# turtle-robotics/sea-current

Hardware: AMD Instinct MI355X
Metric: plans/sec (batched start-goal, 1024^2 grid) (higher is better)
Workload: dtype int32; 1 GPU; 1024x1024 random-obstacle grids (salt20, one grid and one query block per step), EDT + A*, 1024 batched queries per GPU and step, 10 steps = 10240 queries per library call; queries_per_launch=10240, map=salt20, queries_per_gpu=1024, queries_total=1024, lmax=4096, parallelism=query-sharded x1, contexts_in_flight=2, steps_per_call=10, hw_queues=4

## Files before the change

### sea-current_amd/csrc/astar.hip

```cpp
#include "sc_internal.h"
#include <stdlib.h>

#define NBUCKET 32
#ifndef ASTAR_CQ_THROUGHPUT
#define ASTAR_CQ_THROUGHPUT 1024
#define ASTAR_RU_THROUGHPUT 4
#endif
#ifndef ASTAR_CQ_LATENCY
#define ASTAR_CQ_LATENCY 2048
#define ASTAR_RU_LATENCY 8
#endif
#define E_RUN (1u << 18)
#define E_START (4u << 13 | 3u << 16)
#define RUNK 8
#ifndef WIDE_RUNS
#define WIDE_RUNS 0
#endif

struct astar_args {
    const uint8_t* moves;
    const int32_t* d2;
    int W, H;
    int32_t rmin;
    const int32_t* start;
    const int32_t* goal;
    const int32_t* qgrid;
    const int32_t* order;
    const int32_t* nq_dev;
    int nq;
    int Lmax;
    int32_t* path;
    int32_t* len;
    int32_t* cost;
    int32_t* status;
    void* g;
    uint32_t* closed;
    uint32_t* buckets;
    int cap;
    int32_t* expanded;
    int32_t* counter;
    int32_t* ovf_list;
    int32_t* ovf_count;
    int32_t* ovf_sticky;
    int nstat;
    int lazy;
    int tw, bw;
    size_t gcells, bwords;
};

__device__ __forceinline__ int octile(int x, int y, int gx, int gy) {
    int dx = abs(x - gx), dy = abs(y - gy);
    return 10 * max(dx, dy) + 4 * min(dx, dy);
}

__device__ __forceinline__ uint32_t gix(int x, int y, int tw) {
    return ((((uint32_t)(y >> 2) * (uint32_t)tw + (uint32_t)(x >> 2)) << 4) | ((uint32_t)(y & 3) << 2)) | (uint32_t)(x & 3);
}
__device__ __forceinline__ uint32_t gix8(int x, int y, int tw8) {
    return ((((uint32_t)(y >> 3) * (uint32_t)tw8 + (uint32_t)(x >> 3)) << 6) | ((uint32_t)(y & 7) << 3)) | (uint32_t)(x & 7);
}
template <typename GT> __device__ __forceinline__ uint32_t gidx(int x, int y, int tw);
template <> __device__ __forceinline__ uint32_t gidx<uint32_t>(int x, int y, int tw) { return gix(x, y, tw); }
template <> __device__ __forceinline__ uint32_t gidx<uint8_t>(int x, int y, int tw) { return gix8(x, y, tw); }
__device__ __forceinline__ uint32_t cix(int x, int y, int bw) {
    return (((uint32_t)(y >> 4) * (uint32_t)bw + (uint32_t)(x >> 5)) << 4) | (uint32_t)(y & 15);
}

template <typename T>
__device__ __forceinline__ T g_load(const T* p) {
    return __hip_atomic_load(p, __ATOMIC_RELAXED, __HIP_MEMORY_SCOPE_AGENT);
}

__device__ __forceinline__ uint32_t prune_always(int d) {
    const unsigned long long T = 0x75B6D9EA34C851A2ull;
    return (uint32_t)(T >> (8 * d)) & 0xFFu;
}

__device__ __forceinline__ uint32_t entry_pack(int x, int y, int d, uint32_t pmv) {
    const int e0 = (int)((0x6476u >> (4 * (d & 3))) & 7u), e1 = (int)((0x7554u >> (4 * (d & 3))) & 7u);
    const uint32_t side = d < 4 ? (((pmv >> e0) & 1u) | (((pmv >> e1) & 1u) << 1)) : 0u;
    return (uint32_t)y << 19 | side << 16 | (uint32_t)d << 13 | (uint32_t)x;
}
__device__ __forceinline__ uint32_t entry_prune(uint32_t e) {
    const int d = (int)((e >> 13) & 7u);
    uint32_t prune = prune_always(d);
    const int k0 = d < 2 ? 3 : 0, k1 = d < 2 ? 2 : 1;
    const int e0 = (int)((0x6476u >> (4 * (d & 3))) & 7u), e1 = (int)((0x7554u >> (4 * (d & 3))) & 7u);
    if ((e >> 16) & 1u) prune |= (1u << k0) | (1u << e0);
    if ((e >> 17) & 1u) prune |= (1u << k1) | (1u << e1);
    if (e & E_RUN) prune |= 1u << d;
    return (e & 0x3E000u) == E_START ? 0u : prune;
}

__device__ __forceinline__ void masked_atomic_or_issue(uint32_t* addr, uint32_t bits, uint32_t& old) {
    unsigned long long sv;
    asm volatile("s_mov_b64 %[sv], exec\n\t"
                 "v_cmp_ne_u32_e32 vcc, 0, %[b]\n\t"
                 "s_and_b64 exec, %[sv], vcc\n\t"
                 "global_atomic_or %[o], %[a], %[b], off sc0\n\t"
                 "s_mov_b64 exec, %[sv]"
                 : [sv] "=&s"(sv), [o] "+v"(old)
                 : [a] "v"(addr), [b] "v"(bits)
                 : "vcc", "scc", "memory");
}
__device__ __forceinline__ void atomic_wait(uint32_t& old) { asm volatile("s_waitcnt vmcnt(0)" : "+v"(old) : : "memory"); }
__device__ __forceinline__ void pop_pair_issue(const uint8_t* mv_addr, uint32_t* bit_addr, uint32_t bits, uint32_t& pmv, uint32_t& old) {
    unsigned long long sv;
    asm volatile("global_load_ubyte %[m], %[ma], off\n\t"
                 "s_mov_b64 %[sv], exec\n\t"
                 "v_cmp_ne_u32_e32 vcc, 0, %[b]\n\t"
                 "s_and_b64 exec, %[sv], vcc\n\t"
                 "global_atomic_or %[o], %[a], %[b], off sc0\n\t"
                 "s_mov_b64 exec, %[sv]"
                 : [sv] "=&s"(sv), [o] "+v"(old), [m] "=&v"(pmv)
                 : [a] "v"(bit_addr), [b] "v"(bits), [ma] "v"(mv_addr)
                 : "vcc", "scc", "memory");
}
__device__ __forceinline__ void pop_run_issue(const uint8_t* const (&ra)[RUNK - 1], const uint8_t* mv_addr, uint32_t* bit_addr, uint32_t bits,
                                              uint32_t (&rm)[RUNK - 1], uint32_t& pmv, uint32_t& old) {
    static_assert(RUNK == 8, "seven run loads are spelled out");
    unsigned long long sv;
    asm volatile("global_load_ubyte %[r0], %[p0], off\n\t"
                 "global_load_ubyte %[r1], %[p1], off\n\t"
                 "global_load_ubyte %[r2], %[p2], off\n\t"
                 "global_load_ubyte %[r3], %[p3], off\n\t"
                 "global_load_ubyte %[r4], %[p4], off\n\t"
                 "global_load_ubyte %[r5], %[p5], off\n\t"
                 "global_load_ubyte %[r6], %[p6], off\n\t"
                 "global_load_ubyte %[m], %[ma], off\n\t"
                 "s_mov_b64 %[sv], exec\n\t"
                 "v_cmp_ne_u32_e32 vcc, 0, %[b]\n\t"
                 "s_and_b64 exec, %[sv], vcc\n\t"
                 "global_atomic_or %[o], %[a], %[b], off sc0\n\t"
                 "s_mov_b64 exec, %[sv]"
                 : [sv] "=&s"(sv), [o] "+v"(old), [m] "=&v"(pmv), [r0] "=&v"(rm[0]), [r1] "=&v"(rm[1]), [r2] "=&v"(rm[2]), [r3] "=&v"(rm[3]),
                   [r4] "=&v"(rm[4]), [r5] "=&v"(rm[5]), [r6] "=&v"(rm[6])
                 : [a] "v"(bit_addr), [b] "v"(bits), [ma] "v"(mv_addr), [p0] "v"(ra[0]), [p1] "v"(ra[1]), [p2] "v"(ra[2]), [p3] "v"(ra[3]),
                   [p4] "v"(ra[4]), [p5] "v"(ra[5]), [p6] "v"(ra[6])
                 : "vcc", "scc", "memory");
}
__device__ __forceinline__ void pop_run_wait_loads(uint32_t (&rm)[RUNK - 1], uint32_t& pmv, uint32_t& old) {
    asm volatile("s_waitcnt vmcnt(1)" : "+v"(pmv), "+v"(old), "+v"(rm[0]), "+v"(rm[1]), "+v"(rm[2]), "+v"(rm[3]), "+v"(rm[4]), "+v"(rm[5]), "+v"(rm[6]) : : "memory");
}
__device__ __forceinline__ void run_loads_issue(const uint8_t* const (&ra)[RUNK - 1], uint32_t (&rm)[RUNK - 1]) {
    asm volatile("global_load_ubyte %[r0], %[p0], off\n\t"
                 "global_load_ubyte %[r1], %[p1], off\n\t"
                 "global_load_ubyte %[r2], %[p2], off\n\t"
                 "global_load_ubyte %[r3], %[p3], off\n\t"
                 "global_load_ubyte %[r4], %[p4], off\n\t"
                 "global_load_ubyte %[r5], %[p5], off\n\t"
                 "global_load_ubyte %[r6], %[p6], off"
                 : [r0] "=&v"(rm[0]), [r1] "=&v"(rm[1]), [r2] "=&v"(rm[2]), [r3] "=&v"(rm[3]), [r4] "=&v"(rm[4]), [r5] "=&v"(rm[5]), [r6] "=&v"(rm[6])
                 : [p0] "v"(ra[0]), [p1] "v"(ra[1]), [p2] "v"(ra[2]), [p3] "v"(ra[3]), [p4] "v"(ra[4]), [p5] "v"(ra[5]), [p6] "v"(ra[6])
                 : "memory");
}
__device__ __forceinline__ void run_loads_wait(uint32_t (&rm)[RUNK - 1]) {
    asm volatile("s_waitcnt vmcnt(0)" : "+v"(rm[0]), "+v"(rm[1]), "+v"(rm[2]), "+v"(rm[3]), "+v"(rm[4]), "+v"(rm[5]), "+v"(rm[6]) : : "memory");
}
__device__ __forceinline__ void atomic_wait_but(uint32_t& old, uint32_t (&rm)[RUNK - 1]) {
    asm volatile("s_waitcnt vmcnt(7)" : "+v"(old), "+v"(rm[0]), "+v"(rm[1]), "+v"(rm[2]), "+v"(rm[3]), "+v"(rm[4]), "+v"(rm[5]), "+v"(rm[6]) : : "memory");
}
__device__ __forceinline__ void pop_pair_wait_load(uint32_t& pmv, uint32_t& old) { asm volatile("s_waitcnt vmcnt(1)" : "+v"(pmv), "+v"(old) : : "memory"); }

__device__ __forceinline__ void pop_loads_issue(const uint8_t* mv_addr, const uint32_t* w_addr, uint32_t& byte, uint32_t& word) {
    asm volatile("global_load_ubyte %0, %2, off\n\t"
                 "global_load_dword %1, %3, off sc1"
                 : "=&v"(byte), "=&v"(word) : "v"(mv_addr), "v"(w_addr) : "memory");
}
__device__ __forceinline__ void pop_loads_wait(uint32_t& byte, uint32_t& word) { asm volatile("s_waitcnt vmcnt(0)" : "+v"(byte), "+v"(word) : : "memory"); }
__device__ __forceinline__ void masked_or_noret(uint32_t* addr, uint32_t bits) {
    unsigned long long sv;
    asm volatile("s_mov_b64 %[sv], exec\n\t"
                 "v_cmp_ne_u32_e32 vcc, 0, %[b]\n\t"
                 "s_and_b64 exec, %[sv], vcc\n\t"
                 "global_atomic_or %[a], %[b], off\n\t"
                 "s_mov_b64 exec, %[sv]"
                 : [sv] "=&s"(sv) : [a] "v"(addr), [b] "v"(bits) : "vcc", "scc", "memory");
}

__device__ __forceinline__ uint32_t bcast_group8(uint32_t v) {
    const uint32_t q = (uint32_t)__builtin_amdgcn_update_dpp(0, (int)v, 0x00 , 0xF, 0xF, false);
    const uint32_t r = (uint32_t)__builtin_amdgcn_update_dpp(0, (int)q, 0x114 , 0xF, 0xF, false);
    return q | r;
}

#ifdef ASTAR_MARKERS
#define MARK(i, v) do { if (threadIdx.x == 0 && blockIdx.x == 0) __hip_atomic_store(&a.counter[8 + (i)], (int)(v), __ATOMIC_RELAXED, __HIP_MEMORY_SCOPE_SYSTEM); } while (0)
#else
#define MARK(i, v) do { } while (0)
#endif
#ifdef ASTAR_STAMPS
#define STAMP(i) do { const unsigned long long t_ = __builtin_amdgcn_s_memtime(); stamp[i] += (long long)(t_ - t_last); t_last = t_; } while (0)
#else
#define STAMP(i) do { } while (0)
#endif

#ifndef HQ
#define HQ 256
#endif
#define ASTAR_SPIN_LIMIT (1 << 20)
template <typename GT, bool DUAL, int CQ, int REFILL_UNROLL>
__device__ __forceinline__ void astar_query(const astar_args& a, const int q, const int slot) {
    constexpr int REFILL = CQ / 2;
    __shared__ uint32_t qe[CQ + 64];
    __shared__ int s_head[NBUCKET];
    __shared__ int s_tail[NBUCKET];
    __shared__ uint32_t nd_xy[64];
    __shared__ uint32_t nd_mv[64];
    __shared__ uint16_t succ[512];
    __shared__ uint8_t prune_tbl[64];
    __shared__ uint32_t dup_tbl[DUAL ? 1024 + 64 : 1];
    __shared__ uint2 hq_rec[DUAL ? HQ + 64 : 1];
    __shared__ int hq_tail, hq_head, hq_clean, hq_stop, hq_ovf, hq_fcur, hq_found, hq_flush;
    constexpr int SCOPE = DUAL ? __HIP_MEMORY_SCOPE_WORKGROUP : __HIP_MEMORY_SCOPE_WAVEFRONT;
    const int lane = threadIdx.x & 63;
    const int wv = DUAL ? __builtin_amdgcn_readfirstlane((int)(threadIdx.x >> 6)) : 0;
    const int W = a.W, H = a.H;
    const size_t cells = (size_t)W * H;
    const int s = a.start[q], t = a.goal[q];
    int32_t* path = a.path + (size_t)q * a.Lmax;

    int out_st = SC_Q_OK, out_len = 0, out_cost = -1, nexp = 0, npop = 0, kcyc = 0, nstep = 0;
    const size_t grid_off = a.qgrid ? (size_t)a.qgrid[q] * cells : 0;
    const uint8_t* const mvs = a.moves + grid_off;
    const bool bad = s < 0 || t < 0 || (size_t)s >= cells || (size_t)t >= cells || a.d2[grid_off + s] < a.rmin || a.d2[grid_off + t] < a.rmin;
    if (bad) out_st = SC_Q_BAD_ENDPOINT;
    else if (s == t) {
        if (lane == 0 && wv == 0) path[0] = s;
        out_len = 1; out_cost = 0; nexp = 1;
    } else {
    MARK(0, 1);
    const int tw = a.tw, bw = a.bw;
    GT* g = static_cast<GT*>(a.g) + (size_t)slot * a.gcells;
    uint32_t* cl = a.closed + (size_t)slot * a.bwords;
    uint32_t* bk = a.buckets + (size_t)slot * NBUCKET * a.cap;
    const int cap = a.cap, capm = a.cap - 1;
    const int sx = s % W, sy = s / W, gx = t % W, gy = t / W;
    const int ddx[8] = {1, -1, 0, 0, 1, -1, 1, -1};
    const int ddy[8] = {0, 0, 1, -1, 1, 1, -1, -1};

    {
        uint4* p = reinterpret_cast<uint4*>(cl);
        const size_t n4 = a.bwords >> 2;
        for (size_t i = DUAL ? threadIdx.x : lane; i < n4; i += DUAL ? 128 : 64) p[i] = make_uint4(0, 0, 0, 0);
    }
    __builtin_amdgcn_wave_barrier();
    if (wv == 0 && lane < NBUCKET) { s_head[lane] = 0; s_tail[lane] = 0; }
    if (wv == 0) prune_tbl[lane] = (uint8_t)entry_prune((uint32_t)lane << 13);
    if (DUAL)
        for (int i = threadIdx.x; i < 1024 + 64; i += 128) dup_tbl[i] = 0xFFFFFFFFu;
    int fcur = octile(sx, sy, gx, gy);
    if (wv == 0 && lane == 0) {
        qe[0] = (uint32_t)sy << 19 | E_START | (uint32_t)sx;
        hq_tail = 0; hq_head = 0; hq_clean = 0; hq_stop = 0; hq_ovf = 0; hq_fcur = fcur; hq_found = 0; hq_flush = 0;
    }
    asm volatile("s_waitcnt vmcnt(0)" ::: "memory");
    wave_lds_sync();
    if (DUAL) __syncthreads();
    int lh = 0, lt = 1;
    MARK(0, 2);

    bool found = false, ovf = false;
    const unsigned long long t_begin = __builtin_amdgcn_s_memtime();
#ifdef ASTAR_STAMPS
    long long stamp[12] = {0, 0, 0, 0, 0, 0, 0, 0, 0, 0, 0, 0};
    unsigned long long t_last = t_begin;
    int nwide = 0, nrounds = 0, n_qfull = 0, n_lvl = 0, b_batches = 0, b_records = 0, b_idle = 0, n_refill = 0;
#endif
    int steps_left = (int)(8 * cells + 1024 < 0x7FFFFFFF ? 8 * cells + 1024 : 0x7FFFFFFF);

    const int mdx = (int)((0x2252u >> (2 * (lane & 7))) & 3u) - 1;
    const int mdy = (int)((0x0A25u >> (2 * (lane & 7))) & 3u) - 1;
    const uint32_t mw = (lane & 7) < 4 ? 10u : 14u;
    const int moff = mdy * W + mdx;

    auto push_entry = [&](const bool act, const uint32_t ne, const int df) {
        const bool same = act && df == 0;
        const unsigned long long m0 = __ballot(same);
        bool spill = false;
        if (m0) {
            const int cnt = __popcll(m0);
            if (__builtin_expect(lt - lh + cnt <= CQ, 1)) {
                if (same) {
                    const int rank = __builtin_amdgcn_mbcnt_hi((uint32_t)(m0 >> 32), __builtin_amdgcn_mbcnt_lo((uint32_t)m0, 0u));
                    qe[(lt + rank) & (CQ - 1)] = ne;
                }
                lt += cnt;
            } else spill = true;
        }
        if (act && (df != 0 || spill)) {
            const int bb = (fcur + df) & 31;
            const int pos = __hip_atomic_fetch_add(&s_tail[bb], 1, __ATOMIC_RELAXED, SCOPE);
            if (__builtin_expect(pos - __hip_atomic_load(&s_head[bb], __ATOMIC_RELAXED, SCOPE) >= cap, 0)) ovf = true;
            else bk[(size_t)bb * cap + (pos & capm)] = ne;
        }
        lt = __builtin_amdgcn_readfirstlane(lt);
    };
    int hq_tl = 0, hq_hd = 0;
    auto hand_over = [&](const bool rec, const int hx, const int hy, const uint32_t hm, const uint32_t hp) {
        const unsigned long long wm = __ballot(rec);
        if (wm) {
            const int cnt = __popcll(wm);
            int waited = 0;
            while (__builtin_expect(hq_tl + cnt - hq_hd > HQ, 0)) {
                hq_hd = __builtin_amdgcn_readfirstlane(__hip_atomic_load(&hq_head, __ATOMIC_RELAXED, SCOPE));
                if (hq_tl + cnt - hq_hd > HQ) {
                    __builtin_amdgcn_s_sleep(1);
#ifdef ASTAR_STAMPS
                    ++n_qfull;
#endif
                    if (++waited > ASTAR_SPIN_LIMIT) {
                        ovf = true; steps_left = -1;
                        return wm;
                    }
                }
            }
            {
                const int r = (hq_tl + (int)__builtin_amdgcn_mbcnt_hi((uint32_t)(wm >> 32), __builtin_amdgcn_mbcnt_lo((uint32_t)wm, 0u))) & (HQ - 1);
                hq_rec[rec ? r : HQ + lane] = make_uint2((uint32_t)hy << 16 | (uint32_t)hx, hm | hp << 8);
            }
            hq_tl += cnt;
            wave_lds_sync();
            __hip_atomic_store(&hq_tail, hq_tl, __ATOMIC_RELAXED, SCOPE);
        }
        return wm;
    };
    constexpr uint32_t DUP_KEY = 0x1FFF1FFFu, DUP_EMPTY = 0xFFFFFFFFu;
    auto dup_settle = [&](const bool is, const int hx, const int hy, const uint32_t he) {
        const int h = is ? ((hx + 32 * hy) & 1023) : 1024 + lane;
        const uint32_t key = (uint32_t)hy << 16 | (uint32_t)hx;
        const uint32_t mine = key | ((uint32_t)(lane & 7) << 13) | ((uint32_t)(lane >> 3) << 29);
        const uint32_t before = dup_tbl[h];
        __builtin_amdgcn_fence(__ATOMIC_ACQ_REL, "wavefront");
        dup_tbl[h] = mine;
        wave_lds_sync();
        const uint32_t now = dup_tbl[h];
        const bool closed_before = is && before != DUP_EMPTY && ((before ^ key) & DUP_KEY) == 0u;
        int res = closed_before ? 1 : 0;
        if (__ballot(is && now != mine)) {
            if (is && !closed_before && now != mine) res = ((now ^ key) & DUP_KEY) == 0u ? 1 : 2;
            const bool back = res == 2;
            const unsigned long long mb = __ballot(back);
            if (mb) {
                const int c = __popcll(mb);
                if (__builtin_expect(lt - lh + c <= CQ, 1)) {
                    qe[back ? ((lt + (int)__builtin_amdgcn_mbcnt_hi((uint32_t)(mb >> 32), __builtin_amdgcn_mbcnt_lo((uint32_t)mb, 0u))) & (CQ - 1)) : CQ + lane] = he;
                    lt += c;
                } else push_entry(back, he, 0);
                npop -= c;
            }
        }
        wave_lds_sync();
        return res;
    };
    if (DUAL && wv == 1) {
        int hd = 0;
        bool dirty = false;
        for (;;) {
            const int tl = __builtin_amdgcn_readfirstlane(__hip_atomic_load(&hq_tail, __ATOMIC_RELAXED, SCOPE));
            const int stop = __builtin_amdgcn_readfirstlane(__hip_atomic_load(&hq_stop, __ATOMIC_RELAXED, SCOPE));
            wave_lds_sync();
            if (tl == hd) {
                if (dirty) {
                    asm volatile("s_waitcnt vmcnt(0)" ::: "memory");
                    if (lane == 0) __hip_atomic_store(&hq_clean, hd, __ATOMIC_RELAXED, SCOPE);
                    dirty = false;
                }
                if (stop) break;
                __builtin_amdgcn_s_sleep(4);
#ifdef ASTAR_STAMPS
                ++b_idle;
#endif
                continue;
            }
            if (a.lazy && tl - hd < 48 && !stop &&
                __builtin_amdgcn_readfirstlane(__hip_atomic_load(&hq_flush, __ATOMIC_RELAXED, SCOPE)) != tl) {
                __builtin_amdgcn_s_sleep(4);
                continue;
            }
#ifdef ASTAR_STAMPS
            ++b_batches; b_records += min(tl - hd, 64);
#endif
            const int n = min(tl - hd, 64);
            const bool valid = lane < n;
            const int r = (hd + lane) & (HQ - 1);
            const uint2 rec = valid ? hq_rec[r] : make_uint2(0u, 0u);
            const uint32_t xy = rec.x, m = rec.y;
            const uint32_t f = (uint32_t)__builtin_amdgcn_readfirstlane(__hip_atomic_load(&hq_fcur, __ATOMIC_RELAXED, SCOPE));
            hd += n;
            wave_lds_sync();
            if (lane == 0) __hip_atomic_store(&hq_head, hd, __ATOMIC_RELAXED, SCOPE);
            dirty = true;
            const int x = xy & 0xFFFF, y = xy >> 16;
            const int hc = octile(x, y, gx, gy);
            if (valid) g[gidx<GT>(x, y, tw)] = (GT)(f - (uint32_t)hc);
            if (__ballot(valid && x == gx && y == gy) && lane == 0) __hip_atomic_store(&hq_found, 1, __ATOMIC_RELAXED, SCOPE);
            uint32_t mv = m & 0xFFu;
            nd_xy[lane] = xy;
            nd_mv[lane] = ((m >> 8) & 0xFFu) | ((f - (uint32_t)hc) << 8);
            const uint32_t cnt = (uint32_t)__popc(mv);
            int base = 0, total = 0;
#pragma unroll
            for (int bb = 0; bb < 4; ++bb) {
                const unsigned long long mm = __ballot((cnt >> bb) & 1u);
                base += (int)__builtin_amdgcn_mbcnt_hi((uint32_t)(mm >> 32), __builtin_amdgcn_mbcnt_lo((uint32_t)mm, 0u)) << bb;
                total += __popcll(mm) << bb;
            }
            while (mv) {
                const int dd = __ffs((int)mv) - 1;
                mv &= mv - 1;
                succ[base++] = (uint16_t)(lane << 3 | dd);
            }
            wave_lds_sync();
            for (int j0 = 0; j0 < total; j0 += 64) {
                const bool act = j0 + lane < total;
                const uint32_t sd = act ? succ[j0 + lane] : 0u;
                const int par = (int)(sd >> 3), d = (int)(sd & 7u);
                const uint32_t pxy = nd_xy[par], pm = nd_mv[par];
                const int px = pxy & 0xFFFF, py = pxy >> 16;
                const int nx = px + (int)((0x2252u >> (2 * d)) & 3u) - 1, ny = py + (int)((0x0A25u >> (2 * d)) & 3u) - 1;
                const uint32_t fs = (pm >> 8) + (d < 4 ? 10u : 14u) + (uint32_t)octile(nx, ny, gx, gy);
                if (act) {
                    const int bb = (int)(fs & 31u);
                    const int pos = __hip_atomic_fetch_add(&s_tail[bb], 1, __ATOMIC_RELAXED, SCOPE);
                    if (pos - __hip_atomic_load(&s_head[bb], __ATOMIC_RELAXED, SCOPE) >= cap) __hip_atomic_store(&hq_ovf, 1, __ATOMIC_RELAXED, SCOPE);
                    else bk[(size_t)bb * cap + (pos & capm)] = entry_pack(nx, ny, d, pm & 0xFFu);
                }
            }
            wave_lds_sync();
        }
#ifdef ASTAR_STAMPS
        if (lane == 0 && a.Lmax >= 32) { path[16] = b_batches; path[17] = b_records; path[18] = b_idle; }
#endif
    } else {
    for (;;) {
        const int b = fcur & 31;
        const uint32_t* bq = bk + (size_t)b * cap;
        for (;;) {
            if (__builtin_expect(lt == lh, 0)) {
                STAMP(0);
                wave_lds_sync();
                const int hd = __builtin_amdgcn_readfirstlane(__hip_atomic_load(&s_head[b], __ATOMIC_RELAXED, SCOPE));
                const int tl = __builtin_amdgcn_readfirstlane(__hip_atomic_load(&s_tail[b], __ATOMIC_RELAXED, SCOPE));
                if (hd == tl) break;
                const int n = min(tl - hd, REFILL);
                for (int base = lane; base < n; base += 64 * REFILL_UNROLL) {
                    uint32_t chunk[REFILL_UNROLL];
#pragma unroll
                    for (int k = 0; k < REFILL_UNROLL; ++k)
                        if (base + 64 * k < n) chunk[k] = bq[(hd + base + 64 * k) & capm];
#pragma unroll
                    for (int k = 0; k < REFILL_UNROLL; ++k)
                        if (base + 64 * k < n) qe[(lt + base + 64 * k) & (CQ - 1)] = chunk[k];
                }
                lt += n;
                if (lane == 0) __hip_atomic_store(&s_head[b], hd + n, __ATOMIC_RELAXED, SCOPE);
                wave_lds_sync();
                STAMP(10);
#ifdef ASTAR_STAMPS
                ++n_refill;
#endif
            }
            const int n = min(64, lt - lh);
            npop += n; ++nstep;
            STAMP(0);
            if (DUAL && n <= 16) {
                const int kl = n <= 4 ? 3 : n <= 8 ? 2 : n <= 16 ? 1 : 0, KL = 1 << kl, GL = 2 * KL;
                const int sub = lane >> (kl + 1), j = (lane >> kl) & 1, k = lane & (KL - 1);
                const bool valid = sub < n;
                const uint32_t e_raw = qe[(lh + sub) & (CQ - 1)];
                const uint32_t e = valid ? e_raw : 0u;
                lh += n;
                const int x = e & 0x1FFF, y = e >> 19;
                const uint32_t bit = 1u << (x & 31);
                const int dxg = gx - x, dyg = gy - y, adx = abs(dxg), ady = abs(dyg);
                const int dD = 4 + ((dxg < 0 ? 1 : 0) | (dyg < 0 ? 2 : 0));
                const int dS = adx > ady ? (dxg < 0 ? 1 : 0) : (dyg < 0 ? 3 : 2);
                const uint32_t bD = adx >= 1 && ady >= 1 ? 1u << dD : 0u, bS = adx != ady ? 1u << dS : 0u;
                const int d = j ? dS : dD;
                const bool has = valid && (j ? bS : bD) != 0u;
                const int lgeom = j ? abs(adx - ady) : min(adx, ady);
                const int ddx_ = (int)((0x2252u >> (2 * d)) & 3u) - 1, ddy_ = (int)((0x0A25u >> (2 * d)) & 3u) - 1;
                const uint8_t* const addr = mvs + (y * W + x) + (has ? min(k, lgeom - 1) : 0) * (ddy_ * W + ddx_);
                const bool head = valid && j == 0 && k == 0;
                uint32_t old, byte;
                uint32_t* const wa = &cl[cix(x, y, bw)];
                pop_loads_issue(addr, wa, byte, old);
                const uint32_t prune = prune_tbl[(e >> 13) & 63u];
                const int dup = dup_settle(head, x, y, e);
                pop_loads_wait(byte, old);
                const bool link = has && k < lgeom && ((byte >> d) & 1u) && (k > 0 || !((prune >> d) & 1u));
                const unsigned long long lm = __ballot(link);
                const uint32_t grp = (uint32_t)(lm >> (lane & ~(KL - 1))) & ((1u << KL) - 1u);
                const int run = __ffs((int)~grp) - 1;
                const uint32_t ne = entry_pack(x + (k + 1) * ddx_, y + (k + 1) * ddy_, d, byte) | (k + 1 < run ? E_RUN : 0u);
                const bool won1 = head && dup == 0 && !(old & bit);
                masked_or_noret(wa, won1 ? bit : 0u);
                const unsigned long long wm1 = __ballot(won1);
                const bool act = ((wm1 >> (lane & ~(GL - 1))) & 1ull) && k < run;
                {
                    const unsigned long long ma = __ballot(act);
                    if (ma) {
                        const int c = __popcll(ma);
                        if (__builtin_expect(lt - lh + c <= CQ, 1)) {
                            qe[act ? ((lt + (int)__builtin_amdgcn_mbcnt_hi((uint32_t)(ma >> 32), __builtin_amdgcn_mbcnt_lo((uint32_t)ma, 0u))) & (CQ - 1)) : CQ + lane] = ne;
                            lt += c;
                        } else push_entry(act, ne, 0);
                    }
                }
                hand_over(won1, x, y, (byte & ~prune) & ~(bD | bS), byte);
                nexp += __popcll(wm1);
                STAMP(8);
            } else if (!DUAL && n <= 8) {
                const int sub = lane >> 3, d = lane & 7;
                const bool valid = sub < n;
                const uint32_t e = valid ? qe[(lh + sub) & (CQ - 1)] : 0u;
                lh += n;
                const int x = e & 0x1FFF, y = e >> 19;
                const uint32_t bit = 1u << (x & 31);
                uint32_t old = 0, pmv;
                const int hc = octile(x, y, gx, gy);
                const int nx = x + mdx, ny = y + mdy;
                const int df = (int)mw + octile(nx, ny, gx, gy) - hc;
                const int adx = abs(gx - x), ady = abs(gy - y);
                const int lgeom = d >= 4 ? min(adx, ady) : abs(adx - ady);
                const int lmax = valid && df == 0 ? min(RUNK, lgeom) : 1;
                const uint8_t* const cell = mvs + (y * W + x);
                const uint8_t* ra[RUNK - 1];
                uint32_t rm[RUNK - 1];
#pragma unroll
                for (int k = 1; k < RUNK; ++k) ra[k - 1] = cell + min(k, lmax - 1) * moff;
                pop_run_issue(ra, cell, &cl[cix(x, y, bw)], valid && d == 0 ? bit : 0u, rm, pmv, old);
                const uint32_t prune = prune_tbl[(e >> 13) & 63u];
                pop_run_wait_loads(rm, pmv, old);
                const bool cand = valid && (((pmv & ~prune) >> d) & 1u);
                int run = cand ? 1 : 0;
#pragma unroll
                for (int k = 1; k < RUNK; ++k)
                    if (run == k && k < lmax && ((rm[k - 1] >> d) & 1u)) run = k + 1;
                const uint32_t ne = entry_pack(nx, ny, d, pmv) | (run > 1 ? E_RUN : 0u);
                atomic_wait(old);
                old = bcast_group8(old);
                const bool won = valid && !(old & bit);
                push_entry(won && cand, ne, df);
#pragma unroll
                for (int k = 2; k <= RUNK; ++k) {
                    if (__ballot(won && run >= k) == 0) break;
                    push_entry(won && run >= k, entry_pack(x + k * mdx, y + k * mdy, d, rm[k - 2]) | (run > k ? E_RUN : 0u), 0);
                }
                nexp += __popcll(__ballot(won && d == 0));
                if (__ballot(won && x == gx && y == gy)) found = true;
                if (won && d == 0) g[gidx<GT>(x, y, tw)] = (GT)(fcur - hc);
                STAMP(8);
            } else if (DUAL) {
#ifdef ASTAR_STAMPS
                ++nwide;
#endif
                const bool valid = lane < n;
                const uint32_t e_raw = qe[(lh + lane) & (CQ - 1)];
                const uint32_t e = valid ? e_raw : 0u;
                lh += n;
                const int x = e & 0x1FFF, y = e >> 19;
                const uint32_t bit = 1u << (x & 31);
                uint32_t old, pmv;
                uint32_t* const wa = &cl[cix(x, y, bw)];
                pop_loads_issue(mvs + (y * W + x), wa, pmv, old);
                const int dup = dup_settle(valid, x, y, e);
                const uint32_t prune = prune_tbl[(e >> 13) & 63u];
                const int dxg = gx - x, dyg = gy - y, adx = abs(dxg), ady = abs(dyg);
                const int dD = 4 + ((dxg < 0 ? 1 : 0) | (dyg < 0 ? 2 : 0));
                const int dS = adx > ady ? (dxg < 0 ? 1 : 0) : (dyg < 0 ? 3 : 2);
                const uint32_t bD = adx >= 1 && ady >= 1 ? 1u << dD : 0u, bS = adx != ady ? 1u << dS : 0u;
                const int nxD = x + (dxg < 0 ? -1 : 1), nyD = y + (dyg < 0 ? -1 : 1);
                const int nxS = x + (adx > ady ? (dxg < 0 ? -1 : 1) : 0), nyS = y + (adx > ady ? 0 : (dyg < 0 ? -1 : 1));
                pop_loads_wait(pmv, old);
                const uint32_t cand = valid ? (pmv & ~prune) : 0u;
                const uint32_t neD = (uint32_t)nyD << 19 | (uint32_t)dD << 13 | (uint32_t)nxD;
                const uint32_t neS = entry_pack(nxS, nyS, dS, pmv);
                const bool won = valid && dup == 0 && !(old & bit);
                masked_or_noret(wa, won ? bit : 0u);
                {
                    const bool pD = won && (cand & bD), pS = won && (cand & bS);
                    const unsigned long long mD = __ballot(pD), mS = __ballot(pS);
                    const int cD = __popcll(mD), c2 = cD + __popcll(mS);
                    if (c2) {
                        if (__builtin_expect(lt - lh + c2 <= CQ, 1)) {
                            qe[pD ? ((lt + (int)__builtin_amdgcn_mbcnt_hi((uint32_t)(mD >> 32), __builtin_amdgcn_mbcnt_lo((uint32_t)mD, 0u))) & (CQ - 1)) : CQ + lane] = neD;
                            qe[pS ? ((lt + cD + (int)__builtin_amdgcn_mbcnt_hi((uint32_t)(mS >> 32), __builtin_amdgcn_mbcnt_lo((uint32_t)mS, 0u))) & (CQ - 1)) : CQ + lane] = neS;
                            lt += c2;
                        } else {
                            push_entry(pD, neD, 0);
                            push_entry(pS, neS, 0);
                        }
                    }
                }
                nexp += __popcll(hand_over(won, x, y, cand & ~(bD | bS), pmv));
                STAMP(6);
            } else {
                STAMP(0);
                const bool valid = lane < n;
                const uint32_t e = valid ? qe[(lh + lane) & (CQ - 1)] : 0u;
                lh += n;
                const int x = e & 0x1FFF, y = e >> 19;
                const uint32_t bit = 1u << (x & 31);
                uint32_t old = 0, pmv;
                pop_pair_issue(mvs + (y * W + x), &cl[cix(x, y, bw)], valid ? bit : 0u, pmv, old);
                const uint32_t prune = prune_tbl[(e >> 13) & 63u];
                const int hc = octile(x, y, gx, gy);
                STAMP(1);
                pop_pair_wait_load(pmv, old);
                STAMP(2);
                uint32_t mv = valid ? (pmv & ~prune) : 0u;
                nd_xy[lane] = (uint32_t)y << 16 | (uint32_t)x;
                nd_mv[lane] = pmv;
                const uint32_t cnt = (uint32_t)__popc(mv);
                int base = 0, total = 0;
#pragma unroll
                for (int bb = 0; bb < 4; ++bb) {
                    const unsigned long long m = __ballot((cnt >> bb) & 1u);
                    base += (int)__builtin_amdgcn_mbcnt_hi((uint32_t)(m >> 32), __builtin_amdgcn_mbcnt_lo((uint32_t)m, 0u)) << bb;
                    total += __popcll(m) << bb;
                }
                while (mv) {
                    const int dd = __ffs((int)mv) - 1;
                    mv &= mv - 1;
                    succ[base++] = (uint16_t)(lane << 3 | dd);
                }
                wave_lds_sync();
                STAMP(3);
                bool won = false;
#ifdef ASTAR_STAMPS
                ++nwide;
#endif
                for (int j0 = 0; j0 < total; j0 += 64) {
#ifdef ASTAR_STAMPS
                    ++nrounds;
#endif
                    const bool act = j0 + lane < total;
                    const uint32_t sd = act ? succ[j0 + lane] : 0u;
                    const int par = (int)(sd >> 3), d = (int)(sd & 7u);
                    const uint32_t xy = nd_xy[par], pmvp = nd_mv[par];
                    const int px = xy & 0xFFFF, py = xy >> 16;
                    const int ddx_ = (int)((0x2252u >> (2 * d)) & 3u) - 1, ddy_ = (int)((0x0A25u >> (2 * d)) & 3u) - 1;
                    const int nx = px + ddx_, ny = py + ddy_;
                    const int df = (d < 4 ? 10 : 14) + octile(nx, ny, gx, gy) - octile(px, py, gx, gy);
                    const int adx = abs(gx - px), ady = abs(gy - py);
                    const int lgeom = d >= 4 ? min(adx, ady) : abs(adx - ady);
                    const int lmax = WIDE_RUNS && act && df == 0 ? min(RUNK, lgeom) : 1;
                    const int so = ddy_ * W + ddx_;
                    const uint8_t* const cell = mvs + (py * W + px);
                    const uint8_t* ra[RUNK - 1];
                    uint32_t rm[RUNK - 1];
#pragma unroll
                    for (int k = 1; k < RUNK; ++k) ra[k - 1] = cell + min(k, lmax - 1) * so;
                    if (WIDE_RUNS) run_loads_issue(ra, rm);
                    if (j0 == 0) {
                        STAMP(4);
                        if (WIDE_RUNS) atomic_wait_but(old, rm); else atomic_wait(old);
                        STAMP(5);
                        won = valid && !(old & bit);
                        nexp += __popcll(__ballot(won));
                        if (__ballot(won && x == gx && y == gy)) found = true;
                        nd_mv[lane] = pmv | (won ? 0x100u : 0u);
                        wave_lds_sync();
                    }
                    const bool go = act && ((nd_mv[par] >> 8) & 1u);
                    int run = 1;
                    if (WIDE_RUNS) {
                        run_loads_wait(rm);
#pragma unroll
                        for (int k = 1; k < RUNK; ++k)
                            if (run == k && k < lmax && ((rm[k - 1] >> d) & 1u)) run = k + 1;
                    }
                    push_entry(go, entry_pack(nx, ny, d, pmvp) | (run > 1 ? E_RUN : 0u), df);
                    if (WIDE_RUNS) {
#pragma unroll
                        for (int k = 2; k <= RUNK; ++k) {
                            if (__ballot(go && run >= k) == 0) break;
                            push_entry(go && run >= k, entry_pack(px + k * ddx_, py + k * ddy_, d, rm[k - 2]) | (run > k ? E_RUN : 0u), 0);
                        }
                    }
                }
                if (total == 0) {
                    atomic_wait(old);
                    won = valid && !(old & bit);
                    nexp += __popcll(__ballot(won));
                    if (__ballot(won && x == gx && y == gy)) found = true;
                }
                if (won) g[gidx<GT>(x, y, tw)] = (GT)(fcur - hc);
                STAMP(6);
            }
            lt = __builtin_amdgcn_readfirstlane(lt);
            lh = __builtin_amdgcn_readfirstlane(lh);
            nexp = __builtin_amdgcn_readfirstlane(nexp);
            found = __builtin_amdgcn_readfirstlane((int)found) != 0;
            wave_lds_sync();
            MARK(1, steps_left); MARK(2, fcur); MARK(3, nexp); MARK(4, lt - lh);
            if (--steps_left < 0) ovf = true;
            if (__builtin_expect(DUAL ? steps_left < 0 : __ballot(ovf) != 0, 0)) break;
        }
        if (DUAL) {
            STAMP(0);
            if (a.lazy && lane == 0) __hip_atomic_store(&hq_flush, hq_tl, __ATOMIC_RELAXED, SCOPE);
            for (int waited = 0; __builtin_amdgcn_readfirstlane(__hip_atomic_load(&hq_clean, __ATOMIC_RELAXED, SCOPE)) != hq_tl;) {
                __builtin_amdgcn_s_sleep(1);
#ifdef ASTAR_STAMPS
                ++n_lvl;
#endif
                if (++waited > ASTAR_SPIN_LIMIT) { ovf = true; break; }
            }
            wave_lds_sync();
            if (__hip_atomic_load(&hq_ovf, __ATOMIC_RELAXED, SCOPE)) ovf = true;
            if (__builtin_amdgcn_readfirstlane(__hip_atomic_load(&hq_found, __ATOMIC_RELAXED, SCOPE))) found = true;
            STAMP(7);
        }
        if (__ballot(ovf) || found) break;
        const int rh = __hip_atomic_load(&s_head[lane & 31], __ATOMIC_RELAXED, __HIP_MEMORY_SCOPE_WAVEFRONT);
        const int rt = __hip_atomic_load(&s_tail[lane & 31], __ATOMIC_RELAXED, __HIP_MEMORY_SCOPE_WAVEFRONT);
        const uint32_t nonempty = (uint32_t)__ballot(lane < NBUCKET && rh != rt);
        if (nonempty == 0) break;
        const int r0 = (fcur + 1) & 31;
        const uint32_t rot = r0 ? (nonempty >> r0) | (nonempty << (32 - r0)) : nonempty;
        fcur += 1 + (__ffs((int)rot) - 1);
        if (DUAL && lane == 0) __hip_atomic_store(&hq_fcur, fcur, __ATOMIC_RELAXED, SCOPE);
        STAMP(9);
    }
    if (DUAL && lane == 0) __hip_atomic_store(&hq_stop, 1, __ATOMIC_RELAXED, SCOPE);
    }
    if (DUAL) __syncthreads();

    const bool overflow = __ballot(ovf) != 0;
    if (overflow) {
        if (lane == 0 && wv == 0) {
            const int i = atomicAdd(a.ovf_count, 1);
            a.ovf_list[i] = q;
            *a.ovf_sticky = 1;
        }
        out_st = SC_Q_RING_OVERFLOW;
    } else if (!found) {
        out_st = SC_Q_NO_PATH;
    } else {
        STAMP(9);
        asm volatile("s_waitcnt vmcnt(0)" ::: "memory");
        const int Lmax = a.Lmax;
        int cx = gx, cy = gy, L = 1;
        uint32_t gc = (uint32_t)fcur;
        if (lane == 0) path[Lmax - 1] = t;
        bool broken = false;
        const int wox = lane % 7 - 3, woy = lane / 7 - 3;
        const int md = lane & 7;
        const int mdx_ = (int)((0x2252u >> (2 * md)) & 3u) - 1, mdy_ = (int)((0x0A25u >> (2 * md)) & 3u) - 1;
        const uint32_t mw_ = md < 4 ? 10u : 14u;
        while (!broken && (cx != sx || cy != sy)) {
            uint32_t info = 0u, gw = 0u;
            {
                const int nx = cx + wox, ny = cy + woy;
                if (lane < 49 && nx >= 0 && ny >= 0 && nx < W && ny < H) {
                    const uint32_t mvb = mvs[ny * W + nx];
                    const uint32_t cw = g_load(&cl[cix(nx, ny, bw)]);
                    gw = (uint32_t)g_load(&g[gidx<GT>(nx, ny, tw)]);
                    info = mvb | ((cw >> (nx & 31)) & 1u) << 8;
                }
            }
            int ox = 0, oy = 0;
            for (int k = 0; k < 3 && !broken && (cx != sx || cy != sy); ++k) {
                const int src = (oy - mdy_ + 3) * 7 + (ox - mdx_ + 3);
                const uint32_t ni = (uint32_t)__shfl((int)info, src, 64), ng = (uint32_t)__shfl((int)gw, src, 64);
                const bool ok = lane < 8 && ((ni >> md) & 1u) && ((ni >> 8) & 1u) && (GT)ng == (GT)(gc - mw_);
                const unsigned long long m = __ballot(ok);
                if (!m) broken = true;
                else {
                    const int d = __ffsll((long long)m) - 1;
                    cx -= ddx[d]; cy -= ddy[d];
                    ox -= ddx[d]; oy -= ddy[d];
                    gc -= (d < 4 ? 10u : 14u);
                    ++L;
                    if (lane == 0 && L <= Lmax) path[Lmax - L] = cy * W + cx;
                }
            }
        }
        if (broken) out_st = SC_Q_NO_PATH;
        else if (L > Lmax) { out_st = SC_Q_TRUNCATED; out_len = L; out_cost = fcur; }
        else {
            const int shift = Lmax - L;
            if (shift > 0) {
                __builtin_amdgcn_fence(__ATOMIC_RELEASE, "workgroup");
                for (int i = 0; i < L; i += 64) {
                    int v = 0;
                    if (i + lane < L) v = __hip_atomic_load(&path[shift + i + lane], __ATOMIC_RELAXED, __HIP_MEMORY_SCOPE_AGENT);
                    if (i + lane < L) path[i + lane] = v;
                    __builtin_amdgcn_fence(__ATOMIC_RELEASE, "workgroup");
                }
            }
            out_len = L; out_cost = fcur;
        }
        STAMP(11);
    }
    kcyc = (int)((__builtin_amdgcn_s_memtime() - t_begin) >> 10);
#ifdef ASTAR_STAMPS
    if (lane == 0 && wv == 0 && a.Lmax >= 16) {
        for (int i = 0; i < 12; ++i) path[i] = (int)(stamp[i] >> 10);
        path[12] = nwide; path[13] = nrounds; path[14] = n_qfull; path[15] = n_lvl; path[19] = n_refill;
    }
#endif
    }
    if (lane == 0 && wv == 0) {
        a.status[q] = out_st; a.len[q] = out_len; a.cost[q] = out_cost;
        a.expanded[q] = nexp; a.expanded[a.nstat + q] = npop; a.expanded[2 * a.nstat + q] = kcyc; a.expanded[3 * a.nstat + q] = nstep;
    }
}

template <typename GT>
__global__ void __launch_bounds__(64) astar_kernel(astar_args a) {
    const int nq = a.nq_dev ? *a.nq_dev : a.nq;
    for (;;) {
        const int qi = __builtin_amdgcn_readfirstlane(atomicAdd(a.counter, 1)) >> 6;
        if (qi >= nq) break;
        astar_query<GT, false, ASTAR_CQ_THROUGHPUT, ASTAR_RU_THROUGHPUT>(a, a.order ? a.order[qi] : qi, (int)blockIdx.x);
    }
}

template <typename GT, int CQ, int RU>
__global__ void __launch_bounds__(128) astar_kernel_dual(astar_args a) {
    __shared__ int s_qi;
    const int nq = a.nq_dev ? *a.nq_dev : a.nq;
    for (;;) {
        if (threadIdx.x == 0) s_qi = atomicAdd(a.counter, 64) >> 6;
        __syncthreads();
        const int qi = __builtin_amdgcn_readfirstlane(s_qi);
        __syncthreads();
        if (qi >= nq) break;
        astar_query<GT, true, CQ, RU>(a, a.order ? a.order[qi] : qi, (int)blockIdx.x);
        __syncthreads();
    }
}

__global__ void __launch_bounds__(1024) astar_prep_kernel(const int32_t* __restrict__ start, const int32_t* __restrict__ goal, int Q, int W,
                                                          int H, int32_t* __restrict__ order, int32_t* __restrict__ ctr) {
    __shared__ int hist[1024];
    __shared__ int scan[1024];
    const int tid = threadIdx.x;
    if (tid < 4) ctr[tid] = 0;
    if (!order) return;
    hist[tid] = 0;
    __syncthreads();
    const int hmax = 14 * max(W, H) + 1;
    auto key = [&](int q) {
        const int s = start[q], t = goal[q];
        if (s < 0 || t < 0 || s >= W * H || t >= W * H) return 1023;
        const int h = octile(s % W, s / W, t % W, t / W);
        return 1023 - min(1023, (int)(((long long)h * 1024) / hmax));
    };
    for (int q = tid; q < Q; q += 1024) atomicAdd(&hist[key(q)], 1);
    __syncthreads();
    scan[tid] = hist[tid];
    __syncthreads();
    for (int o = 1; o < 1024; o <<= 1) {
        const int v = tid >= o ? scan[tid - o] : 0;
        __syncthreads();
        scan[tid] += v;
        __syncthreads();
    }
    hist[tid] = scan[tid] - hist[tid];
    __syncthreads();
    for (int q = tid; q < Q; q += 1024) order[atomicAdd(&hist[key(q)], 1)] = q;
}

__global__ void __launch_bounds__(256) gfield_kernel(const uint32_t* g, const uint32_t* cl, int W, int H, int tw, int bw, uint32_t* out) {
    size_t i = (size_t)blockIdx.x * 256 + threadIdx.x;
    if (i < (size_t)W * H) {
        const int x = (int)(i % W), y = (int)(i / W);
        out[i] = (cl[cix(x, y, bw)] >> (x & 31)) & 1u ? g[gix(x, y, tw)] : 0xFFFFFFFFu;
    }
}

static int astar_resident_waves(sc_ctx* ctx) {
    if (ctx->astar_waves > 0) return ctx->astar_waves;
    int per_cu = 0, dev = ctx->device;
    hipDeviceProp_t prop;
    if (hipOccupancyMaxActiveBlocksPerMultiprocessor(&per_cu, astar_kernel<uint8_t>, 64, 0) != hipSuccess || per_cu <= 0) per_cu = 8;
    if (hipGetDeviceProperties(&prop, dev) != hipSuccess || prop.multiProcessorCount <= 0) prop.multiProcessorCount = 256;
    int w = per_cu * prop.multiProcessorCount;
    if (const char* e = getenv("SC_ASTAR_WAVES")) { const int v = atoi(e); if (v > 0) w = v; }
    ctx->astar_waves = w;
    return w;
}
static int astar_resident_dual(sc_ctx* ctx, bool latency) {
    int& cached = latency ? ctx->astar_dual_lat : ctx->astar_dual;
    if (cached >= 0) return cached;
    int per_cu = 0, n = 0;
    hipDeviceProp_t prop;
    const hipError_t e_ = latency ? hipOccupancyMaxActiveBlocksPerMultiprocessor(&per_cu, astar_kernel_dual<uint8_t, ASTAR_CQ_LATENCY, ASTAR_RU_LATENCY>, 128, 0)
                                  : hipOccupancyMaxActiveBlocksPerMultiprocessor(&per_cu, astar_kernel_dual<uint8_t, ASTAR_CQ_THROUGHPUT, ASTAR_RU_THROUGHPUT>, 128, 0);
    if (e_ == hipSuccess && per_cu > 0 && hipGetDeviceProperties(&prop, ctx->device) == hipSuccess && prop.multiProcessorCount > 0)
        n = per_cu * prop.multiProcessorCount;
    if (const char* e = getenv("SC_ASTAR_DUAL")) { const int v = atoi(e); if (v == 0) n = 0; else if (v > 1 && v < n) n = v; }
    if (latency) { if (const char* e = getenv("SC_ASTAR_LATENCY")) { if (atoi(e) == 0) n = 0; } }
    cached = n;
    return n;
}

static int astar_run(sc_ctx* ctx, const int32_t* d2, int G, const int32_t* qgrid, int W, int H, int32_t r2, const int32_t* start,
                     const int32_t* goal, int Q, int Lmax, int32_t* path, int32_t* len, int32_t* cost,
                     int32_t* status, bool full_g = false) {
    const size_t cells = (size_t)W * H;
    const int tw = full_g ? (W + 3) >> 2 : (W + 7) >> 3, bw = (W + 31) >> 5;
    const size_t gcells = full_g ? (size_t)tw * ((H + 3) >> 2) * 16 : (size_t)tw * ((H + 7) >> 3) * 64;
    const size_t gsz = full_g ? 4 : 1;
    const size_t bwords = (size_t)bw * ((H + 15) >> 4) * 16;
    const int32_t rmin = r2 > 1 ? r2 : 1;
    int r = sc_scratch_reserve(ctx, &ctx->moves, cells * (size_t)G);
    if (r != SC_OK) return r;
    r = sc_launch_moves(ctx, d2, W, H * G, H, r2, (uint8_t*)ctx->moves.p);
    if (r != SC_OK) return r;
    r = sc_scratch_reserve(ctx, &ctx->qstats, (size_t)Q * 6 * sizeof(int32_t));
    if (r != SC_OK) return r;
    int32_t* expanded = (int32_t*)ctx->qstats.p;
    int32_t* order = expanded + 4 * (size_t)Q;
    int32_t* ovf_list = order + Q;
    ctx->last_Q = Q;
    int cap = ctx->astar_cap;
    if (const char* e = getenv("SC_ASTAR_CAP")) { const int v = atoi(e); if (v >= 1024 && (v & (v - 1)) == 0) cap = v; }
    if (cells > ((size_t)1 << 21)) {
        int want = 1 << 15;
        while (want < 64 * (W > H ? W : H)) want <<= 1;
        if (cap < want) cap = want;
    }
    const size_t per_slot = gcells * gsz + bwords * 4 + (size_t)NBUCKET * cap * 4;
    size_t slots = ctx->astar_slot_budget / per_slot;
    const size_t rlat = (size_t)astar_resident_dual(ctx, true);
    const bool latency = !full_g && rlat > 0 && (size_t)Q <= rlat && (size_t)Q <= slots;
    const size_t rdual = latency ? rlat : (size_t)astar_resident_dual(ctx, false);
    const bool dual = !full_g && rdual > 0;
    const size_t resident = dual ? rdual : (size_t)astar_resident_waves(ctx);
    if (slots > resident) slots = resident;
    if (slots > (size_t)Q) slots = Q;
    if (slots < 1) slots = 1;
    auto ring_slots = [](size_t n) { return n > 16 ? n : (size_t)16; };
    if (slots * gcells * gsz > ctx->gslots.bytes || slots * bwords * 4 > ctx->closed.bytes || ring_slots(slots) * NBUCKET * (size_t)cap * 4 > ctx->buckets.bytes) {
        size_t free_b = 0, total_b = 0;
        if (hipMemGetInfo(&free_b, &total_b) == hipSuccess) {
            const size_t avail = (size_t)(0.9 * (double)(free_b + ctx->gslots.bytes + ctx->closed.bytes + ctx->buckets.bytes));
            while (slots > 1 && slots * (gcells * gsz + bwords * 4) + ring_slots(slots) * NBUCKET * (size_t)cap * 4 > avail) slots = (slots + 1) / 2;
        }
    }
    for (;;) {
        r = sc_scratch_reserve(ctx, &ctx->gslots, slots * gcells * gsz);
        if (r == SC_OK) r = sc_scratch_reserve(ctx, &ctx->closed, slots * bwords * 4);
        if (r == SC_OK) r = sc_scratch_reserve(ctx, &ctx->buckets, ring_slots(slots) * NBUCKET * (size_t)cap * 4);
        if (r == SC_OK) break;
        if (r != SC_ERR_NOMEM || slots <= 1) return r;
        (void)hipGetLastError();
        slots = (slots + 1) / 2;
    }
    if (!ctx->actr.p) {
        r = sc_scratch_reserve(ctx, &ctx->actr, 16 * sizeof(int32_t));
        if (r != SC_OK) return r;
        SC_HIP(ctx, hipMemsetAsync(ctx->actr.p, 0, 16 * sizeof(int32_t), ctx->stream));
    }
    int32_t* ctr = (int32_t*)ctx->actr.p;

    const bool sorted = (size_t)Q > slots;
    int tk = sc_time_begin(ctx, SC_K_ASTAR);
    hipLaunchKernelGGL(astar_prep_kernel, dim3(1), dim3(1024), 0, ctx->stream, start, goal, Q, W, H, sorted ? order : (int32_t*)nullptr, ctr);
    astar_args a{(const uint8_t*)ctx->moves.p, d2, W, H, rmin, start, goal, qgrid, sorted ? order : nullptr, nullptr, Q, Lmax, path, len,
                 cost, status, ctx->gslots.p, (uint32_t*)ctx->closed.p, (uint32_t*)ctx->buckets.p, cap, expanded, ctr,
                 ovf_list, ctr + 1, ctr + 4, Q, (dual && (size_t)Q > slots) ? 1 : 0, tw, bw, gcells, bwords};
    if (full_g) hipLaunchKernelGGL(astar_kernel<uint32_t>, dim3((unsigned)slots), dim3(64), 0, ctx->stream, a);
    else if (dual && latency && (size_t)Q <= slots)
        hipLaunchKernelGGL((astar_kernel_dual<uint8_t, ASTAR_CQ_LATENCY, ASTAR_RU_LATENCY>), dim3((unsigned)slots), dim3(128), 0, ctx->stream, a);
    else if (dual)
        hipLaunchKernelGGL((astar_kernel_dual<uint8_t, ASTAR_CQ_THROUGHPUT, ASTAR_RU_THROUGHPUT>), dim3((unsigned)slots), dim3(128), 0, ctx->stream, a);
    else hipLaunchKernelGGL(astar_kernel<uint8_t>, dim3((unsigned)slots), dim3(64), 0, ctx->stream, a);
    {
        const size_t rslots = slots >= 16 ? slots / 16 : 1;
        const int rcap = cap * 16;
        astar_args b = a;
        b.order = ovf_list; b.nq_dev = ctr + 1; b.nq = 0; b.cap = rcap; b.counter = ctr + 2;
        b.ovf_list = order; b.ovf_count = ctr + 3;
        if (full_g) hipLaunchKernelGGL(astar_kernel<uint32_t>, dim3((unsigned)rslots), dim3(64), 0, ctx->stream, b);
        else hipLaunchKernelGGL(astar_kernel<uint8_t>, dim3((unsigned)rslots), dim3(64), 0, ctx->stream, b);
    }
    sc_time_end(ctx, tk);
    SC_HIP(ctx, hipGetLastError());
    return SC_OK;
}

extern "C" int sc_astar_batch(sc_ctx* ctx, const int32_t* d2, int W, int H, int32_t r2_clear,
                              const int32_t* start, const int32_t* goal, int Q, int Lmax,
                              int32_t* path, int32_t* len, int32_t* cost, int32_t* status) {
    if (!ctx || !d2 || !start || !goal || !path || !len || !cost || !status || W <= 0 || H <= 0 || Q < 0 ||
        Lmax <= 0 || W > SC_MAX_DIM || H > SC_MAX_DIM)
        return SC_ERR_INVALID;
    if (Q == 0) return SC_OK;
    SC_HIP(ctx, hipSetDevice(ctx->device));
    return astar_run(ctx, d2, 1, nullptr, W, H, r2_clear, start, goal, Q, Lmax, path, len, cost, status);
}

extern "C" int sc_astar_batch_multi(sc_ctx* ctx, const int32_t* d2, int G, const int32_t* qgrid, int W, int H, int32_t r2_clear,
                                    const int32_t* start, const int32_t* goal, int Q, int Lmax,
                                    int32_t* path, int32_t* len, int32_t* cost, int32_t* status) {
    if (!ctx || !d2 || !qgrid || !start || !goal || !path || !len || !cost || !status || G <= 0 || W <= 0 || H <= 0 || Q < 0 ||
        Lmax <= 0 || W > SC_MAX_DIM || H > SC_MAX_DIM || (long long)H * G > 0x7FFFFFFF / (W > 0 ? W : 1))
        return SC_ERR_INVALID;
    if (Q == 0) return SC_OK;
    SC_HIP(ctx, hipSetDevice(ctx->device));
    return astar_run(ctx, d2, G, qgrid, W, H, r2_clear, start, goal, Q, Lmax, path, len, cost, status);
}

extern "C" int sc_astar_last_expansions(sc_ctx* ctx, int64_t* expansions) {
    if (!ctx || !expansions) return SC_ERR_INVALID;
    *expansions = 0;
    if (ctx->last_Q <= 0) return SC_OK;
    std::vector<int32_t> ex(ctx->last_Q);
    SC_HIP(ctx, hipMemcpyAsync(ex.data(), ctx->qstats.p, (size_t)ctx->last_Q * 4, hipMemcpyDeviceToHost, ctx->stream));
    SC_HIP(ctx, hipStreamSynchronize(ctx->stream));
    int64_t tot = 0;
    for (int v : ex) tot += v;
    *expansions = tot;
    return SC_OK;
}

extern "C" int sc_astar_gfield(sc_ctx* ctx, const int32_t* d2, int W, int H, int32_t r2_clear,
                               int32_t start, int32_t goal, uint32_t* gfield, int32_t* cost, int32_t* status) {
    if (!ctx || !d2 || !gfield || !cost || !status || W <= 0 || H <= 0 || W > SC_MAX_DIM || H > SC_MAX_DIM)
        return SC_ERR_INVALID;
    SC_HIP(ctx, hipSetDevice(ctx->device));
    const size_t cells = (size_t)W * H;
    int r = sc_scratch_reserve(ctx, &ctx->staging[7], 64);
    if (r != SC_OK) return r;
    int32_t* sg = (int32_t*)ctx->staging[7].p;
    int32_t h[2] = {start, goal};
    SC_HIP(ctx, hipMemcpyAsync(sg, h, 8, hipMemcpyHostToDevice, ctx->stream));
    SC_HIP(ctx, hipStreamSynchronize(ctx->stream));
    r = astar_run(ctx, d2, 1, nullptr, W, H, r2_clear, sg, sg + 1, 1, 1, sg + 4, sg + 2, cost, status, true);
    if (r != SC_OK) return r;
    hipLaunchKernelGGL(gfield_kernel, dim3((unsigned)((cells + 255) / 256)), dim3(256), 0, ctx->stream,
                       (const uint32_t*)ctx->gslots.p, (const uint32_t*)ctx->closed.p, W, H, (W + 3) >> 2, (W + 31) >> 5, gfield);
    SC_HIP(ctx, hipGetLastError());
    return SC_OK;
}

extern "C" int sc_astar_debug_peek(sc_ctx* ctx, int32_t* out16) {
    if (!ctx || !out16 || !ctx->actr.p) return SC_ERR_INVALID;
    hipStream_t s;
    SC_HIP(ctx, hipStreamCreateWithFlags(&s, hipStreamNonBlocking));
    SC_HIP(ctx, hipMemcpyAsync(out16, ctx->actr.p, 16 * sizeof(int32_t), hipMemcpyDeviceToHost, s));
    SC_HIP(ctx, hipStreamSynchronize(s));
    SC_HIP(ctx, hipStreamDestroy(s));
    return SC_OK;
}

extern "C" int sc_astar_debug_stats(sc_ctx* ctx, int32_t* out, int Q) {
    if (!ctx || !out || Q != ctx->last_Q) return SC_ERR_INVALID;
    SC_HIP(ctx, hipMemcpyAsync(out, ctx->qstats.p, (size_t)Q * 16, hipMemcpyDeviceToHost, ctx->stream));
    SC_HIP(ctx, hipStreamSynchronize(ctx->stream));
    return SC_OK;
}
```

Measured before the change: 660,400 plans/s.

## Read kernel args from kernarg segment and simplify overflow/step-limit handling

```diff
diff --git a/sea-current_amd/csrc/astar.hip b/sea-current_amd/csrc/astar.hip
--- a/sea-current_amd/csrc/astar.hip
+++ b/sea-current_amd/csrc/astar.hip
@@ -195,12 +195,17 @@
 #define STAMP(i) do { } while (0)
 #endif
 
+typedef __attribute__((address_space(4))) const astar_args karg_t;
+__device__ __forceinline__ karg_t* karg_reload(karg_t* p) { asm volatile("" : "+s"(p)); return p; }
+__device__ __forceinline__ karg_t* karg_ptr() { return karg_reload((karg_t*)__builtin_amdgcn_kernarg_segment_ptr()); }
+
 #ifndef HQ
 #define HQ 256
 #endif
 #define ASTAR_SPIN_LIMIT (1 << 20)
 template <typename GT, bool DUAL, int CQ, int REFILL_UNROLL>
-__device__ __forceinline__ void astar_query(const astar_args& a, const int q, const int slot) {
+__device__ __forceinline__ void astar_query(karg_t* const ka, const int q, const int slot) {
+    karg_t& a = *ka;
     constexpr int REFILL = CQ / 2;
     __shared__ uint32_t qe[CQ + 64];
     __shared__ int s_head[NBUCKET];
@@ -267,7 +272,7 @@
     unsigned long long t_last = t_begin;
     int nwide = 0, nrounds = 0, n_qfull = 0, n_lvl = 0, b_batches = 0, b_records = 0, b_idle = 0, n_refill = 0;
 #endif
-    int steps_left = (int)(8 * cells + 1024 < 0x7FFFFFFF ? 8 * cells + 1024 : 0x7FFFFFFF);
+    const int step_limit = (int)(8 * cells + 1024 < 0x7FFFFFFF ? 8 * cells + 1024 : 0x7FFFFFFF);
 
     const int mdx = (int)((0x2252u >> (2 * (lane & 7))) & 3u) - 1;
     const int mdy = (int)((0x0A25u >> (2 * (lane & 7))) & 3u) - 1;
@@ -291,10 +296,20 @@
         if (act && (df != 0 || spill)) {
             const int bb = (fcur + df) & 31;
             const int pos = __hip_atomic_fetch_add(&s_tail[bb], 1, __ATOMIC_RELAXED, SCOPE);
-            if (__builtin_expect(pos - __hip_atomic_load(&s_head[bb], __ATOMIC_RELAXED, SCOPE) >= cap, 0)) ovf = true;
+            if (__builtin_expect(pos - __hip_atomic_load(&s_head[bb], __ATOMIC_RELAXED, SCOPE) >= cap, 0)) {
+                if (DUAL) __hip_atomic_store(&hq_ovf, 1, __ATOMIC_RELAXED, SCOPE);
+                else ovf = true;
+            } else bk[(size_t)bb * cap + (pos & capm)] = ne;
+        }
+        lt = __builtin_amdgcn_readfirstlane(lt);
+    };
+    auto park_entry = [&](const bool act, const uint32_t ne) {
+        if (act) {
+            const int bb = fcur & 31;
+            const int pos = __hip_atomic_fetch_add(&s_tail[bb], 1, __ATOMIC_RELAXED, SCOPE);
+            if (__builtin_expect(pos - __hip_atomic_load(&s_head[bb], __ATOMIC_RELAXED, SCOPE) >= cap, 0)) __hip_atomic_store(&hq_ovf, 1, __ATOMIC_RELAXED, SCOPE);
             else bk[(size_t)bb * cap + (pos & capm)] = ne;
         }
-        lt = __builtin_amdgcn_readfirstlane(lt);
     };
     int hq_tl = 0, hq_hd = 0;
     auto hand_over = [&](const bool rec, const int hx, const int hy, const uint32_t hm, const uint32_t hp) {
@@ -310,7 +325,7 @@
                     ++n_qfull;
 #endif
                     if (++waited > ASTAR_SPIN_LIMIT) {
-                        ovf = true; steps_left = -1;
+                        ovf = true;
                         return wm;
                     }
                 }
@@ -346,7 +361,8 @@
                 if (__builtin_expect(lt - lh + c <= CQ, 1)) {
                     qe[back ? ((lt + (int)__builtin_amdgcn_mbcnt_hi((uint32_t)(mb >> 32), __builtin_amdgcn_mbcnt_lo((uint32_t)mb, 0u))) & (CQ - 1)) : CQ + lane] = he;
                     lt += c;
-                } else push_entry(back, he, 0);
+                } else if (DUAL) park_entry(back, he);
+                else push_entry(back, he, 0);
                 npop -= c;
             }
         }
@@ -505,7 +521,7 @@
                         if (__builtin_expect(lt - lh + c <= CQ, 1)) {
                             qe[act ? ((lt + (int)__builtin_amdgcn_mbcnt_hi((uint32_t)(ma >> 32), __builtin_amdgcn_mbcnt_lo((uint32_t)ma, 0u))) & (CQ - 1)) : CQ + lane] = ne;
                             lt += c;
-                        } else push_entry(act, ne, 0);
+                        } else park_entry(act, ne);
                     }
                 }
                 hand_over(won1, x, y, (byte & ~prune) & ~(bD | bS), byte);
@@ -589,8 +605,8 @@
                             qe[pS ? ((lt + cD + (int)__builtin_amdgcn_mbcnt_hi((uint32_t)(mS >> 32), __builtin_amdgcn_mbcnt_lo((uint32_t)mS, 0u))) & (CQ - 1)) : CQ + lane] = neS;
                             lt += c2;
                         } else {
-                            push_entry(pD, neD, 0);
-                            push_entry(pS, neS, 0);
+                            park_entry(pD, neD);
+                            park_entry(pS, neS);
                         }
                     }
                 }
@@ -695,9 +711,9 @@
             nexp = __builtin_amdgcn_readfirstlane(nexp);
             found = __builtin_amdgcn_readfirstlane((int)found) != 0;
             wave_lds_sync();
-            MARK(1, steps_left); MARK(2, fcur); MARK(3, nexp); MARK(4, lt - lh);
-            if (--steps_left < 0) ovf = true;
-            if (__builtin_expect(DUAL ? steps_left < 0 : __ballot(ovf) != 0, 0)) break;
+            MARK(1, nstep); MARK(2, fcur); MARK(3, nexp); MARK(4, lt - lh);
+            if (nstep > step_limit) ovf = true;
+            if (__builtin_expect(DUAL ? ovf : __ballot(ovf) != 0, 0)) break;
         }
         if (DUAL) {
             STAMP(0);
@@ -710,7 +726,7 @@
                 if (++waited > ASTAR_SPIN_LIMIT) { ovf = true; break; }
             }
             wave_lds_sync();
-            if (__hip_atomic_load(&hq_ovf, __ATOMIC_RELAXED, SCOPE)) ovf = true;
+            if (__builtin_amdgcn_readfirstlane(__hip_atomic_load(&hq_ovf, __ATOMIC_RELAXED, SCOPE))) ovf = true;
             if (__builtin_amdgcn_readfirstlane(__hip_atomic_load(&hq_found, __ATOMIC_RELAXED, SCOPE))) found = true;
             STAMP(7);
         }
@@ -811,26 +827,30 @@
 }
 
 template <typename GT>
-__global__ void __launch_bounds__(64) astar_kernel(astar_args a) {
-    const int nq = a.nq_dev ? *a.nq_dev : a.nq;
+__global__ void __launch_bounds__(64) astar_kernel(astar_args) {
+    karg_t* const ka = karg_ptr();
+    const int nq = ka->nq_dev ? *ka->nq_dev : ka->nq;
     for (;;) {
+        karg_t& a = *karg_reload(ka);
         const int qi = __builtin_amdgcn_readfirstlane(atomicAdd(a.counter, 1)) >> 6;
         if (qi >= nq) break;
-        astar_query<GT, false, ASTAR_CQ_THROUGHPUT, ASTAR_RU_THROUGHPUT>(a, a.order ? a.order[qi] : qi, (int)blockIdx.x);
+        astar_query<GT, false, ASTAR_CQ_THROUGHPUT, ASTAR_RU_THROUGHPUT>(&a, a.order ? a.order[qi] : qi, (int)blockIdx.x);
     }
 }
 
 template <typename GT, int CQ, int RU>
-__global__ void __launch_bounds__(128) astar_kernel_dual(astar_args a) {
+__global__ void __launch_bounds__(128) astar_kernel_dual(astar_args) {
     __shared__ int s_qi;
-    const int nq = a.nq_dev ? *a.nq_dev : a.nq;
+    karg_t* const ka = karg_ptr();
+    const int nq = ka->nq_dev ? *ka->nq_dev : ka->nq;
     for (;;) {
+        karg_t& a = *karg_reload(ka);
         if (threadIdx.x == 0) s_qi = atomicAdd(a.counter, 64) >> 6;
         __syncthreads();
         const int qi = __builtin_amdgcn_readfirstlane(s_qi);
         __syncthreads();
         if (qi >= nq) break;
-        astar_query<GT, true, CQ, RU>(a, a.order ? a.order[qi] : qi, (int)blockIdx.x);
+        astar_query<GT, true, CQ, RU>(&a, a.order ? a.order[qi] : qi, (int)blockIdx.x);
         __syncthreads();
     }
 }
```

After: 661,100 plans/s (median of 6 runs). Within noise of the previous version (+0.1%).
